# cmhungsteve/TA3N

Measured on AMD Instinct MI355X. Metric: src+tgt videos/sec per train step, UCF->HMDB_full 5-seg TA3N, higher is better.
Workload: dtype bf16

## Files before the change

### ta3n_amd/csrc/ta3n_gemm_kernel.h

```cpp
#pragma once
#include <hip/hip_runtime.h>
#include <cstdlib>
#include <cstring>

#include <type_traits>

#include "ta3n_kernels.h"

using namespace ta3n;

namespace {

typedef float f32x16 __attribute__((ext_vector_type(16)));
typedef __attribute__((address_space(3))) void lds_void_t;

constexpr int BKC = 64;

__device__ __forceinline__ float4 zero4() { return make_float4(0.f, 0.f, 0.f, 0.f); }

__device__ __forceinline__ void glds16(const float *gsrc, unsigned lds_byte_addr) {
    unsigned keep;
    lds_byte_addr = __builtin_amdgcn_readfirstlane(lds_byte_addr);
    asm volatile("s_mov_b32 %0, m0\n\ts_mov_b32 m0, %2\n\ts_nop 0\n\tglobal_load_lds_dwordx4 %1, off\n\ts_mov_b32 m0, %0"
                 : "=&s"(keep) : "v"(gsrc), "s"(lds_byte_addr) : "memory");
// ... 464 lines not shown
                    acc = __builtin_amdgcn_mfma_f32_32x32x8bf16_1k(__builtin_bit_cast(s16x4, AH), __builtin_bit_cast(s16x4, BH), acc, 0, 0, 0);
                }
            }
        }
        return;
    }
    if (BF) {
        if (NQ % 2 == 0) {
#pragma unroll
            for (int q = 0; q < NQ; q += 2) {
                if (FULL || 4 * (wk * GPW + 2 * q) < krem) {
                    const u32x4 a = {pack_bf16(av[q][0], av[q][1]), pack_bf16(av[q][2], av[q][3]),
                                     pack_bf16(av[q + 1][0], av[q + 1][1]), pack_bf16(av[q + 1][2], av[q + 1][3])};
                    const u32x4 b = {pack_bf16(bv[q][0], bv[q][1]), pack_bf16(bv[q][2], bv[q][3]),
                                     pack_bf16(bv[q + 1][0], bv[q + 1][1]), pack_bf16(bv[q + 1][2], bv[q + 1][3])};
                    acc = __builtin_amdgcn_mfma_f32_32x32x16_bf16(__builtin_bit_cast(bf16x8, a), __builtin_bit_cast(bf16x8, b),
                                                                  acc, 0, 0, 0);
                }
            }
        } else {
#pragma unroll
            for (int q = 0; q < NQ; ++q) {
                if (FULL || 4 * (wk * GPW + 2 * q) < krem) {
                    const u32x2 a = {pack_bf16(av[q][0], av[q][1]), pack_bf16(av[q][2], av[q][3])};
                    const u32x2 b = {pack_bf16(bv[q][0], bv[q][1]), pack_bf16(bv[q][2], bv[q][3])};
                    acc = __builtin_amdgcn_mfma_f32_32x32x8bf16_1k(__builtin_bit_cast(s16x4, a), __builtin_bit_cast(s16x4, b), acc,
                                                                   0, 0, 0);
                }
            }
        }
        return;
    }
#pragma unroll
    for (int q = 0; q < NQ; ++q) {
        if (FULL || 4 * (wk * GPW + 2 * q) < krem) {
#pragma unroll
            for (int j = 0; j < 4; ++j) acc = __builtin_amdgcn_mfma_f32_32x32x2f32(av[q][j], bv[q][j], acc, 0, 0, 0);
        }
    }
}

__device__ __forceinline__ void st_pub(float *p, f32x4 v) { asm volatile("global_store_dwordx4 %0, %1, off sc0 sc1" ::"v"(p), "v"(v) : "memory"); }
__device__ __forceinline__ void st_pub(void *p, u32x2 v) { asm volatile("global_store_dwordx2 %0, %1, off sc0 sc1" ::"v"(p), "v"(v) : "memory"); }
__device__ __forceinline__ void st_pub(float *p, float v) { asm volatile("global_store_dword %0, %1, off sc0 sc1" ::"v"(p), "v"(v) : "memory"); }
__device__ __forceinline__ void st_pub(unsigned short *p, unsigned v) { asm volatile("global_store_short %0, %1, off sc0 sc1" ::"v"(p), "v"(v) : "memory"); }

__device__ __forceinline__ void store_twin4(unsigned short *tp, unsigned w0, unsigned w1, int nrem, bool vec, bool pub) {
    if (nrem >= 4 && vec) {
        if (pub) st_pub(tp, u32x2{w0, w1});
        else *reinterpret_cast<u32x2 *>(tp) = u32x2{w0, w1};
    } else {
        const unsigned short h[4] = {(unsigned short)(w0 & 0xFFFF), (unsigned short)(w0 >> 16), (unsigned short)(w1 & 0xFFFF), (unsigned short)(w1 >> 16)};
#pragma unroll
        for (int e = 0; e < 4; ++e)
            if (e < nrem) { if (pub) st_pub(tp + e, (unsigned)h[e]); else tp[e] = h[e]; }
    }
}

constexpr int CHAIN_SPIN_LIMIT = 1 << 20;
__device__ __forceinline__ void chain_wait(const Task &t, const Wait *__restrict__ waits, int *__restrict__ cnt, int tid, int knobs) {
    const int nwait = (knobs & 1024) ? 0 : t.wait_count;
    if (nwait > 0) {
        if (tid < 64) {
            for (int w0 = 0; w0 < nwait; w0 += 64) {
                const bool mine = w0 + tid < nwait;
                Wait w{0, 0};
                if (mine) w = waits[t.wait_begin + w0 + tid];
                bool ok = !mine;
                int spins = 0;
                for (;;) {
                    if (!ok) ok = ((knobs & 2048) ? __hip_atomic_fetch_add(cnt + 2 + w.counter, 0, __ATOMIC_RELAXED, __HIP_MEMORY_SCOPE_AGENT)
                                                  : __hip_atomic_load(cnt + 2 + w.counter, __ATOMIC_RELAXED, __HIP_MEMORY_SCOPE_AGENT)) >= w.target;
                    if (__all(ok)) break;
                    if (++spins > CHAIN_SPIN_LIMIT) {
                        if (tid == 0) __hip_atomic_store(cnt + 1, 1 + (int)blockIdx.x, __ATOMIC_RELAXED, __HIP_MEMORY_SCOPE_AGENT);
                        break;
                    }
                    if ((spins & 1023) == 0 && __hip_atomic_load(cnt + 1, __ATOMIC_RELAXED, __HIP_MEMORY_SCOPE_AGENT) != 0) break;
                    for (int z = 0; z < (knobs & 255); ++z) __builtin_amdgcn_s_sleep(8);
                }
            }
            if (!(knobs & 256)) __builtin_amdgcn_fence(__ATOMIC_ACQUIRE, "agent");
        }
        __syncthreads();
    }
}
__device__ __forceinline__ void chain_exit(int sig, int *__restrict__ cnt, int n_counters, int tid, int knobs) {
    if ((knobs & 512) && sig < 0) return;
    asm volatile("s_waitcnt vmcnt(0)" ::: "memory");
    __syncthreads();
    if (tid == 0) {
        if (knobs & 512) { __hip_atomic_fetch_add(cnt + 2 + sig, 1, __ATOMIC_RELAXED, __HIP_MEMORY_SCOPE_AGENT); return; }
        if (sig >= 0) {
            const int before = __hip_atomic_fetch_add(cnt + 2 + sig, 1, __ATOMIC_RELAXED, __HIP_MEMORY_SCOPE_AGENT);
            asm volatile("s_waitcnt vmcnt(0)" ::"v"(before) : "memory");
        }
        const int done = __hip_atomic_fetch_add(cnt, 1, __ATOMIC_RELAXED, __HIP_MEMORY_SCOPE_AGENT);
        if (done == (int)gridDim.x - 1) {
            for (int i = 0; i < n_counters; ++i) __hip_atomic_store(cnt + 2 + i, 0, __ATOMIC_RELAXED, __HIP_MEMORY_SCOPE_AGENT);
            __hip_atomic_store(cnt, 0, __ATOMIC_RELAXED, __HIP_MEMORY_SCOPE_AGENT);
        }
    }
}

__device__ __forceinline__ const float *base_ptr(const Ptrs &p, int base) {
    switch (base) {
        case BASE_X: return p.x;
        case BASE_P: return p.p;
        case BASE_G: return p.g;
        case BASE_P16: return p.p16;
        default: return p.ws;
    }
}

}

#ifdef TA3N_GEMM_STAMPS
#define TA3N_STAMP_SLOTS 16
#define TA3N_STAMP_FLOATS (8192 * TA3N_STAMP_SLOTS * 2)
#define GSTAMP_PTR (reinterpret_cast<unsigned long long *>(const_cast<float *>(ptrs.ws) + zeros_off - TA3N_STAMP_FLOATS))
#define GSTAMP(i) do { if (threadIdx.x == 0 && blockIdx.x < 8192) GSTAMP_PTR[blockIdx.x * TA3N_STAMP_SLOTS + (i)] = __builtin_amdgcn_s_memtime(); } while (0)
#define GSTAMP_VAL(i, v) do { if (threadIdx.x == 0 && blockIdx.x < 8192) GSTAMP_PTR[blockIdx.x * TA3N_STAMP_SLOTS + (i)] = (unsigned long long)(v); } while (0)
#define GSTAMP_W1(i, v) do { if (threadIdx.x == 64 && blockIdx.x < 8192) GSTAMP_PTR[blockIdx.x * TA3N_STAMP_SLOTS + (i)] = (unsigned long long)(v); } while (0)
#define FSTAMP_DECL unsigned long long ks_f0 = __builtin_amdgcn_s_memtime(), ks_f[4] = {0, 0, 0, 0}, ks_e = 0
#define FSTAMP(i, dep) do { asm volatile("" ::"s"(dep)); ks_f[i] = (__builtin_amdgcn_s_memtime() - ks_f0) & 0xFFFFull; } while (0)
#define ESTAMP(a, b, c) do { asm volatile("" ::"s"(a), "s"(b), "s"(c)); ks_e = __builtin_amdgcn_s_memtime(); } while (0)
#define KSTAMP_DECL unsigned long long ks_wait = 0, ks_comp = 0, ks_t = 0, ks_bnd = 0, ks_int = 0, ks_mfull = 0, ks_mlast = 0, ks_m0 = 0; int ks_n = 0
#define KSTAMP_ISSUED(acc) do { acc += (__builtin_amdgcn_s_memtime() - ks_t) + (1ull << 40); } while (0)
#define KSTAMP_COMP_BEGIN do { ks_m0 = __builtin_amdgcn_s_memtime(); } while (0)
#define KSTAMP_COMP_DONE(acc) do { acc += (__builtin_amdgcn_s_memtime() - ks_m0) + (1ull << 40); } while (0)
#define KSTAMP_BEGIN_WAIT do { ks_t = __builtin_amdgcn_s_memtime(); } while (0)
#define KSTAMP_END_WAIT do { const unsigned long long n_ = __builtin_amdgcn_s_memtime(); ks_wait += n_ - ks_t; ks_t = n_; ++ks_n; } while (0)
#define KSTAMP_END_COMP do { if (ks_t != 0) { const unsigned long long n_ = __builtin_amdgcn_s_memtime(); ks_comp += n_ - ks_t; } } while (0)
#else
#define GSTAMP(i) do { } while (0)
#define GSTAMP_VAL(i, v) do { } while (0)
#define FSTAMP_DECL ((void)0)
#define FSTAMP(i, dep) ((void)0)
#define ESTAMP(a, b, c) ((void)0)
#define KSTAMP_DECL do { } while (0)
#define KSTAMP_BEGIN_WAIT do { } while (0)
#define KSTAMP_END_WAIT do { } while (0)
#define KSTAMP_END_COMP do { } while (0)
#define KSTAMP_ISSUED(acc) do { } while (0)
#define KSTAMP_COMP_BEGIN do { } while (0)
#define KSTAMP_COMP_DONE(acc) do { } while (0)
#endif

#ifndef TA3N_SEG_FAST
#define TA3N_SEG_FAST 1
#endif
#ifndef TA3N_TASK_FAST
#define TA3N_TASK_FAST 1
#endif

#define TASK_F(f) (TASK_LANES ? static_cast<decltype(t.f)>(__builtin_amdgcn_readlane(tv, (int)(offsetof(Task, f) / 4))) : t.f)
#define TASK_A(a, i) (TASK_LANES ? __builtin_amdgcn_readlane(tv, (int)(offsetof(Task, a) / 4) + (i)) : t.a[i])
#define HYPER_F(f) (TASK_LANES ? __builtin_bit_cast(float, __builtin_amdgcn_readlane(hv, (int)(offsetof(Hyper, f) / 4))) : hh.f)
#define HYPER_U(f) (TASK_LANES ? (uint32_t)__builtin_amdgcn_readlane(hv, (int)(offsetof(Hyper, f) / 4)) : hh.f)

namespace ta3n {

template <int WM, int WN, int WK, int BF, int NS, int RM, int RN, int KV = 63>
__device__ __forceinline__ void gemm_tile(const Task &t, const Seg *__restrict__ segs, const Ptrs &ptrs, int hyper_off, int zeros_off,
                                          int twin_off, const SgdSide &side, int pair_delta, int knobs) {
    constexpr int NW = WM * WN * WK, NT = 64 * NW;
    constexpr int BM = 32 * WM * RM, BN = 32 * WN * RN;
    constexpr bool HS = BF == 5;
    constexpr int ROWF = HS ? BKC / 2 : BKC;
    constexpr int STAGE = (BM + BN) * ROWF;
    constexpr int CH = BF == 2 ? 2 * BKC : BKC;
    constexpr bool TW = BF == 2 || BF == 4 || BF == 5;
    constexpr bool PAIR = BF == 4;
    constexpr int EPI = NW * RM * RN * 32 * 36;
    constexpr int LDS_FLOATS = NS * STAGE > EPI + 4 ? NS * STAGE : EPI + 4;
    __shared__ __attribute__((aligned(16))) float lds[LDS_FLOATS];

    const int tid = threadIdx.x, lane = tid & 63;
    const int wave = __builtin_amdgcn_readfirstlane(tid >> 6);
    const unsigned lds_base = __builtin_amdgcn_readfirstlane((unsigned)(uintptr_t)(lds_void_t *)lds);
    const int li = lane & 31, lh = lane >> 5;
    const int wk = wave % WK, wn = (wave / WK) % WN, wm = wave / (WK * WN);

    GSTAMP(0);
    FSTAMP_DECL;
    constexpr bool TASK_LANES = TA3N_EXPERIMENTS == 0 && KV != 63 && (TA3N_TASK_FAST) != 0;
    static_assert(sizeof(Task) == 200 && sizeof(Task) / 4 <= 64, "a Task is 50 dwords: one per lane of a wave");
    static_assert(offsetof(Hyper, train) / 4 == 19, "the per-step scalars the tiles use are the first 20 dwords of Hyper");
    int tv = 0, hv = 0;
    if constexpr (TASK_LANES) {
        __builtin_memcpy(&tv, reinterpret_cast<const char *>(&t) + 4 * (lane < (int)(sizeof(Task) / 4) ? lane : 0), 4);
        __builtin_memcpy(&hv, reinterpret_cast<const char *>(ptrs.ws + hyper_off) + 4 * (lane < 20 ? lane : 0), 4);
        asm volatile("" ::"v"(tv), "v"(hv));
    }
    FSTAMP(0, TASK_F(epi));
    auto task_seg0 = [&]() -> Seg {
        Seg s;
        s.a_base = TASK_F(seg0.a_base); s.b_base = TASK_F(seg0.b_base); s.a_off = TASK_F(seg0.a_off); s.b_off = TASK_F(seg0.b_off);
        s.a_ld = TASK_F(seg0.a_ld); s.b_ld = TASK_F(seg0.b_ld); s.a_kmajor = TASK_F(seg0.a_kmajor); s.b_kmajor = TASK_F(seg0.b_kmajor);
        s.klen = TASK_F(seg0.klen); s.scale_kind = TASK_F(seg0.scale_kind); s.pad[0] = TASK_A(seg0.pad, 0); s.pad[1] = TASK_A(seg0.pad, 1);
        return s;
    };
    constexpr bool OPT = TA3N_EXPERIMENTS != 0 && (KV & 32) != 0;
    const bool pub = OPT && TASK_F(sig) >= 0 && !(side.p16_off == -12345);
    if (TASK_F(epi) & EPI_SGD) {
        if (side.params == nullptr) return;
        float part = 0.f;
        if (tid < 256)
            part = strided_partial_sum(ptrs.ws + side.norm_off, side.norm_n, tid, 256);
        part = wave_allreduce_sum(part);
        if (lane == 0 && wave < 4) lds[wave] = part;
        __syncthreads();
        const float total = sqrtf(((lds[0] + lds[1]) + lds[2]) + lds[3]);
        const float coef = clip_coef(total, side.clip);
        float4 *__restrict__ p4 = reinterpret_cast<float4 *>(side.params);
        float4 *__restrict__ m4 = reinterpret_cast<float4 *>(side.momentum);
        const float4 *__restrict__ g4 = reinterpret_cast<const float4 *>(ptrs.g);
        for (int i = TASK_A(pad, 0) + tid; i < TASK_A(pad, 1); i += NT) {
            const float4 p = p4[i], m = m4[i], gr = g4[i];
            float gg[4] = {gr.x, gr.y, gr.z, gr.w}, pp[4] = {p.x, p.y, p.z, p.w}, mm[4] = {m.x, m.y, m.z, m.w};
#pragma unroll
            for (int e = 0; e < 4; ++e) nesterov_sgd(pp[e], mm[e], gg[e] * coef, side.lr, side.mu, side.wd);
            if (pub) st_pub(reinterpret_cast<float *>(p4 + i), f32x4{pp[0], pp[1], pp[2], pp[3]});
            else p4[i] = make_float4(pp[0], pp[1], pp[2], pp[3]);
            m4[i] = make_float4(mm[0], mm[1], mm[2], mm[3]);
            if (side.p16_off >= 0) {
                uint2 *tw = reinterpret_cast<uint2 *>(ptrs.ws + side.p16_off) + i;
                const unsigned h0 = pack_bf16(pp[0], pp[1]), h1 = pack_bf16(pp[2], pp[3]);
                if (pub) st_pub(tw, u32x2{h0, h1});
                else *tw = make_uint2(h0, h1);
                if ((BF == 3 || BF == 4) && pair_delta) {
                    const u32x2 l = {pack_bf16_lo(pp[0], pp[1], h0), pack_bf16_lo(pp[2], pp[3], h1)};
                    if (pub) st_pub(tw + pair_delta / 2, l);
                    else tw[pair_delta / 2] = make_uint2(l[0], l[1]);
                }
            }
        }
        return;
    }
    if (TASK_F(epi) & EPI_COLSUM) {
        float *__restrict__ dst = const_cast<float *>(base_ptr(ptrs, TASK_F(c_base))) + (size_t)TASK_F(c_off);
        const float *__restrict__ src = ptrs.ws + TASK_A(pad, 0);
        float sq = 0.f;
        for (int n = TASK_F(n0) + tid; n < TASK_F(n_valid); n += NT) {
            float v = 0.f;
            const float *__restrict__ col = src + n;
            const int R = TASK_A(pad, 1);
            const size_t ld = (size_t)TASK_A(pad, 2);
            int r = 0;
#pragma unroll 1
            for (; r + 8 <= R; r += 8) {
                float x[8];
#pragma unroll
                for (int i = 0; i < 8; ++i) x[i] = col[(size_t)(r + i) * ld];
#pragma unroll
                for (int i = 0; i < 8; ++i) v += x[i];
            }
            for (; r < R; ++r) v += col[(size_t)r * ld];
            dst[n] = v;
            sq = fmaf(v, v, sq);
            if (OPT && side.p_new != nullptr && TASK_F(c_base) == BASE_G) {
                const size_t pi = (size_t)TASK_F(c_off) + n;
                float p1 = ptrs.p[pi], mm = side.momentum[pi];
                nesterov_sgd(p1, mm, v, side.lr, side.mu, side.wd);
                side.p_new[pi] = p1; side.momentum[pi] = mm;
                if (side.p16_new != nullptr) reinterpret_cast<unsigned short *>(side.p16_new)[pi] = (unsigned short)(pack_bf16(p1, 0.f) & 0xFFFF);
            }
        }
        if (TASK_F(epi) & EPI_SUMSQ) {
            sq = wave_allreduce_sum(sq);
            if (lane == 0) lds[wave] = sq;
            __syncthreads();
            if (tid == 0) {
                float tot = 0.f;
                for (int i = 0; i < NW; ++i) tot += lds[i];
                ptrs.ws[TASK_A(pad, 3)] = tot;
            }
        }
        return;
    }
    if (TASK_F(seg_count) == 0) return;
    if (TASK_F(epi) & EPI_SUMROWS8) {
        const float *__restrict__ src = ptrs.ws + TASK_A(pad, 1);
        float sacc = 0.f;
        for (int r = tid >> 3; r < TASK_A(pad, 2); r += NT / 8) sacc += src[r * 8 + (tid & 7)];
        lds[tid] = sacc;
        __syncthreads();
        if (tid < 8) {
            float v = 0.f;
            for (int i = 0; i < NT / 8; ++i) v += lds[i * 8 + tid];
            ptrs.ws[TASK_A(pad, 0) + tid] = v;
        }
        __syncthreads();
    }
    const Hyper *__restrict__ hy = reinterpret_cast<const Hyper *>(ptrs.ws + hyper_off);
    const float *__restrict__ zeros = ptrs.ws + zeros_off;
    const uint32_t epi = TASK_F(epi);
    struct HyperHead { float beta[3], gamma, lr, momentum, weight_decay, clip, p_drop_i, p_drop_v; uint32_t seed_i, seed_v; };
    const HyperHead hh = TASK_LANES ? HyperHead{} : *reinterpret_cast<const HyperHead *>(hy);
    const int h_train_mem = TASK_LANES ? 0 : hy->train;
#define HYPER_TRAIN (TASK_LANES ? __builtin_amdgcn_readlane(hv, (int)(offsetof(Hyper, train) / 4)) : h_train_mem)
    FSTAMP(1, TASK_LANES ? 0 : h_train_mem);
    auto scale_of = [&](int kind) -> float {
        switch (kind) {
            case SK_NEG_BETA_REL: return -HYPER_F(beta[0]);
            case SK_NEG_BETA_VID: return -HYPER_F(beta[1]);
// ... 255 lines not shown
                    compute_stage<BM, BN, WK, AKM, BKM, true, RS, BF, RM, RN>(acc, rs, sa, sa + BM * ROWF, ra, rb, wk, lh, CH);
                    KSTAMP_COMP_DONE(ks_mfull);
                    buf ^= 1;
                }
                stage_ready();
                const int krem = klen - (n_chunks - 1) * CH, c_scale = scale;
                ++cseg;
                const bool more = cseg < seg_end;
                if (more) {
                    open_seg(cseg);
                    issue(buf ^ 1, 0);
                    KSTAMP_ISSUED(ks_bnd);
                }
                const float *sa = lds + buf * STAGE;
                KSTAMP_COMP_BEGIN;
                compute_stage<BM, BN, WK, AKM, BKM, false, RS, BF, RM, RN>(acc, rs, sa, sa + BM * ROWF, ra, rb, wk, lh, krem);
                if (krem == CH) KSTAMP_COMP_DONE(ks_mlast);
                if (c_scale != SK_ONE) {
                    const float sc = scale_of(c_scale);
    #pragma unroll
                    for (int i = 0; i < RM; ++i)
    #pragma unroll
                        for (int j = 0; j < RN; ++j)
    #pragma unroll
                            for (int r = 0; r < 16; ++r) acc[i][j][r] *= sc;
                }
                if (cseg >= seg_end) break;
                buf ^= 1;
            }
            } else {
            OperandStream<BM, NW, TW, PAIR, HS> oa;
            OperandStream<BN, NW, TW, PAIR, HS> ob;
            constexpr int LPW = OperandStream<BM, NW, TW, PAIR, HS>::NP + OperandStream<BN, NW, TW, PAIR, HS>::NP;
            int i_seg = cseg, i_chunk = 0, i_nchunks = 0, i_klen = 0, i_buf = 0, ahead = 0;
            Seg nx = TASK_LANES ? task_seg0() : t.seg0;
            auto open_issue_seg = [&]() {
                const Seg sg = nx;
                if (i_seg + 1 < seg_end) nx = segs[i_seg + 1];
                i_klen = sg.klen; i_nchunks = (sg.klen + CH - 1) / CH; i_chunk = 0;
                oa.setup(base_ptr(ptrs, sg.a_base) + (size_t)sg.a_off, sg.a_ld, AKM, sg.klen, m0, sg.pad[0] > 0 ? sg.pad[0] : m_valid,
                         wave, lane, pair_delta);
                ob.setup(base_ptr(ptrs, sg.b_base) + (size_t)sg.b_off, sg.b_ld, BKM, sg.klen, n0, n_valid, wave, lane, pair_delta);
            };
            auto issue_one = [&]() {
                const unsigned st = lds_base + (unsigned)(i_buf * STAGE * 4);
                const int k0 = i_chunk * CH;
                oa.issue(k0, i_klen - k0, st, wave, lane, zeros);
                ob.issue(k0, i_klen - k0, st + BM * ROWF * 4, wave, lane, zeros);
                i_buf = (i_buf + 1 == NS) ? 0 : i_buf + 1;
                ++ahead;
                if (++i_chunk == i_nchunks) {
                    if (++i_seg < seg_end) open_issue_seg();
                }
            };
            auto wait_landed = [&](int younger) {
                static_assert((NS - 2) * LPW <= 63, "vmcnt is a 6-bit counter");
                KSTAMP_END_COMP;
                KSTAMP_BEGIN_WAIT;
                if (NS == 2 || younger == 0) asm volatile("s_waitcnt vmcnt(0)" ::: "memory");
                else if (NS == 3 || younger == 1) asm volatile("s_waitcnt vmcnt(%0)" ::"n"(LPW) : "memory");
                else if (NS == 4 || younger == 2) asm volatile("s_waitcnt vmcnt(%0)" ::"n"(2 * LPW) : "memory");
                else if (NS == 5 || younger == 3) asm volatile("s_waitcnt vmcnt(%0)" ::"n"(3 * LPW) : "memory");
                else asm volatile("s_waitcnt vmcnt(%0)" ::"n"(4 * LPW) : "memory");
                __builtin_amdgcn_s_barrier();
                asm volatile("" ::: "memory");
                KSTAMP_END_WAIT;
            };
            open_issue_seg();
    #pragma unroll 1
            for (int sidx = 0; sidx < NS - 1 && i_seg < seg_end; ++sidx) issue_one();
            FSTAMP(3, 0);

            int c_buf = 0;
            int c_klen_nx = TASK_F(seg0.klen), c_scale_nx = TASK_F(seg0.scale_kind);
            for (;;) {
                const int klen = c_klen_nx, c_scale = c_scale_nx;
                if (cseg + 1 < seg_end) { c_klen_nx = segs[cseg + 1].klen; c_scale_nx = segs[cseg + 1].scale_kind; }
                const int n_chunks = (klen + CH - 1) / CH;
                int c = 0;
                if (i_seg == cseg) {
                    for (; c + (NS - 1) < n_chunks; ++c) {
                        wait_landed(NS - 2);
                        const unsigned st = lds_base + (unsigned)(i_buf * STAGE * 4);
                        const int k0 = (c + NS - 1) * CH;
                        const float *sa = lds + c_buf * STAGE;
                        oa.issue(k0, klen - k0, st, wave, lane, zeros);
                        ob.issue(k0, klen - k0, st + BM * ROWF * 4, wave, lane, zeros);
                        KSTAMP_ISSUED(ks_int);
                        KSTAMP_COMP_BEGIN;
                        compute_stage<BM, BN, WK, AKM, BKM, true, RS, BF, RM, RN>(acc, rs, sa, sa + BM * ROWF, ra, rb, wk, lh, CH);
                        KSTAMP_COMP_DONE(ks_mfull);
                        i_buf = (i_buf + 1 == NS) ? 0 : i_buf + 1;
                        c_buf = (c_buf + 1 == NS) ? 0 : c_buf + 1;
                    }
                    if (++i_seg < seg_end) open_issue_seg();
                }
    #pragma unroll 1
                for (; c < n_chunks; ++c) {
                    wait_landed(ahead - 1);
#ifdef TA3N_GEMM_STAMPS
                    const bool ks_first = i_chunk == 0;
                    const int ks_ahead = ahead;
#endif
                    if (i_seg < seg_end) issue_one();
#ifdef TA3N_GEMM_STAMPS
                    if (ahead == ks_ahead) { }
                    else if (ks_first) KSTAMP_ISSUED(ks_bnd);
                    else KSTAMP_ISSUED(ks_int);
#endif
                    const float *sa = lds + c_buf * STAGE;
                    KSTAMP_COMP_BEGIN;
                    if (c < n_chunks - 1)
                        compute_stage<BM, BN, WK, AKM, BKM, true, RS, BF, RM, RN>(acc, rs, sa, sa + BM * ROWF, ra, rb, wk, lh, CH);
                    else
                        compute_stage<BM, BN, WK, AKM, BKM, false, RS, BF, RM, RN>(acc, rs, sa, sa + BM * ROWF, ra, rb, wk, lh, klen - c * CH);
#ifdef TA3N_GEMM_STAMPS
                    if (c < n_chunks - 1) KSTAMP_COMP_DONE(ks_mfull);
                    else if (klen - c * CH == CH) KSTAMP_COMP_DONE(ks_mlast);
#endif
                    c_buf = (c_buf + 1 == NS) ? 0 : c_buf + 1;
                    --ahead;
                }
                if (c_scale != SK_ONE) {
                    const float sc = scale_of(c_scale);
    #pragma unroll
                    for (int i = 0; i < RM; ++i)
    #pragma unroll
                        for (int j = 0; j < RN; ++j)
    #pragma unroll
                            for (int r = 0; r < 16; ++r) acc[i][j][r] *= sc;
                }
                if (++cseg >= seg_end) break;
            }
            }
    };
    using T_ = std::true_type;
    using F_ = std::false_type;
    {
        switch (TASK_F(seg0.a_kmajor) * 2 + TASK_F(seg0.b_kmajor)) {
            case 0: if constexpr (KVE & 1) k_loop(F_{}, F_{}, F_{}); break;
            case 1: if constexpr (KVE & 2) k_loop(F_{}, T_{}, F_{}); break;
            case 2: if constexpr (KVE & 4) k_loop(T_{}, F_{}, F_{}); break;
            default:
                if (TASK_F(epi) & EPI_ROWSUM_A) { if constexpr (KVE & 16) k_loop(T_{}, T_{}, T_{}); }
                else { if constexpr (KVE & 8) k_loop(T_{}, T_{}, F_{}); }
                break;
        }
    }

    KSTAMP_END_COMP;
    GSTAMP(2);
#ifdef TA3N_GEMM_STAMPS
    GSTAMP_VAL(8, ks_wait); GSTAMP_VAL(9, ks_comp); GSTAMP_VAL(10, ks_n);
    GSTAMP_VAL(12, ks_bnd); GSTAMP_VAL(13, ks_int); GSTAMP_VAL(14, ks_mfull); GSTAMP_VAL(15, ks_mlast);
#endif
    __syncthreads();
    GSTAMP(3);
#pragma unroll
    for (int i = 0; i < RM; ++i)
#pragma unroll
        for (int j = 0; j < RN; ++j) {
            float *cs = lds + ((wave * RM + i) * RN + j) * (32 * 36);
#pragma unroll
            for (int r = 0; r < 16; ++r) {
                const int row = (r & 3) + 8 * (r >> 2) + 4 * lh;
                cs[row * 36 + li] = acc[i][j][r];
            }
        }
    __syncthreads();
    GSTAMP(4);

    const float *__restrict__ split_other = nullptr;
    if (OPT && (epi & EPI_SPLITK)) {
        int &split_ticket = *reinterpret_cast<int *>(&lds[EPI]);
        const int half = TASK_A(pad, 2) - 1;
        float *mine = ptrs.ws + TASK_A(pad, 0) + (size_t)half * (BM * BN);
        constexpr int ITER_S = (BM * BN / 4 + NT - 1) / NT;
#pragma unroll
        for (int it = 0; it < ITER_S; ++it) {
            const int idx = tid + it * NT;
            if (idx < BM * BN / 4) {
                const int r = idx / (BN / 4), c4 = (idx % (BN / 4)) * 4;
                const int br = r >> 5, bc = c4 >> 5;
                const int slot0 = ((((br / RM) * WN + (bc / RN)) * WK) * RM + (br % RM)) * RN + (bc % RN);
                float4 v4 = zero4();
#pragma unroll
                for (int q = 0; q < WK; ++q) {
                    const float4 part = *reinterpret_cast<const float4 *>(&lds[(slot0 + q * RM * RN) * (32 * 36) + (r & 31) * 36 + (c4 & 31)]);
                    v4.x += part.x; v4.y += part.y; v4.z += part.z; v4.w += part.w;
                }
                st_pub(mine + (size_t)r * BN + c4, f32x4{v4.x, v4.y, v4.z, v4.w});
            }
        }
        asm volatile("s_waitcnt vmcnt(0)" ::: "memory");
        __syncthreads();
        int *ticket = reinterpret_cast<int *>(ptrs.ws + TASK_A(pad, 1));
        if (tid == 0) split_ticket = __hip_atomic_fetch_add(ticket, 1, __ATOMIC_RELAXED, __HIP_MEMORY_SCOPE_AGENT);
        __syncthreads();
        if (split_ticket == 0) return;
        if (tid == 0) __hip_atomic_store(ticket, 0, __ATOMIC_RELAXED, __HIP_MEMORY_SCOPE_AGENT);
        split_other = ptrs.ws + TASK_A(pad, 0) + (size_t)(1 - half) * (BM * BN);
    }
    const float alpha = scale_of(TASK_F(alpha_kind));
    const float gamma = scale_of(TASK_F(gamma_kind));
    const bool drop_on = (epi & (EPI_DROP_I | EPI_DROP_V)) && HYPER_TRAIN != 0;
    const uint32_t dseed = (epi & EPI_DROP_I) ? HYPER_U(seed_i) : HYPER_U(seed_v);
    const float dp = (epi & EPI_DROP_I) ? HYPER_F(p_drop_i) : HYPER_F(p_drop_v);
    const uint32_t doff = drop_on ? (uint32_t)TASK_F(pad2) : 0u;
    float *__restrict__ cbase = const_cast<float *>(base_ptr(ptrs, TASK_F(c_base))) + (size_t)TASK_F(c_off);
    const EpiOperands eo = PF_IT > 0 ? eo_early : epi_operands();
    const int nfan = eo.nfan;
    const bool c_vec = ((TASK_F(c_off) | TASK_F(c_ld)) & 3) == 0;
    const bool upd = OPT && side.p_new != nullptr && TASK_F(c_base) == BASE_G;
    float sumsq = 0.f;
    ESTAMP(alpha, gamma, TASK_F(c_ld));
    constexpr int ITER = (BM * BN / 4 + NT - 1) / NT;
    constexpr int UNR = ITER <= 4 ? ITER : 2;
#pragma unroll UNR
    for (int it = 0; it < ITER; ++it) {
        const int idx = tid + it * NT;
        if (idx >= BM * BN / 4) break;
        const int r = idx / (BN / 4);
        const int c4 = (idx % (BN / 4)) * 4;
        const int br = r >> 5, bc = c4 >> 5;
        const int slot0 = ((((br / RM) * WN + (bc / RN)) * WK) * RM + (br % RM)) * RN + (bc % RN);
        const int m = m0 + r, n = n0 + c4;
        const bool row_ok = m < m_valid;
        const int nrem = row_ok ? n_valid - n : 0;
        float av[4] = {0.f, 0.f, 0.f, 0.f}, mv[4] = {1.f, 1.f, 1.f, 1.f};
        float fm[3][4] = {{0.f, 0.f, 0.f, 0.f}, {0.f, 0.f, 0.f, 0.f}, {0.f, 0.f, 0.f, 0.f}};
        if constexpr (PF_IT > 0) {
#pragma unroll
            for (int e = 0; e < 4; ++e) { av[e] = add_e[PF_IT > 0 ? it : 0][e]; mv[e] = aux_e[PF_IT > 0 ? it : 0][e]; asm volatile("" : "+v"(mv[e])); }
        } else {
            fetch_add_aux(eo, av, mv, m, n, nrem);
        }
        if constexpr (PF_FAN) {
#pragma unroll
            for (int f = 0; f < 3; ++f)
#pragma unroll
                for (int e = 0; e < 4; ++e) { fm[f][e] = fan_e[f][e]; asm volatile("" : "+v"(fm[f][e])); }
        } else if constexpr (EPI_EARLY) {
            fetch_fan(eo, fm, m, n, nrem);
        }
        float up[4] = {0.f, 0.f, 0.f, 0.f}, um[4] = {0.f, 0.f, 0.f, 0.f};
        if (upd_early) {
#pragma unroll
            for (int e = 0; e < 4; ++e) { up[e] = up_e[UPD_PREFETCH ? it : 0][e]; um[e] = um_e[UPD_PREFETCH ? it : 0][e]; }
        } else if (upd && nrem > 0) {
            const size_t pi = (size_t)TASK_F(c_off) + (size_t)m * TASK_F(c_ld) + n;
            if (nrem >= 4 && c_vec) {
                const float4 q4 = *reinterpret_cast<const float4 *>(ptrs.p + pi), r4 = *reinterpret_cast<const float4 *>(side.momentum + pi);
                up[0] = q4.x; up[1] = q4.y; up[2] = q4.z; up[3] = q4.w; um[0] = r4.x; um[1] = r4.y; um[2] = r4.z; um[3] = r4.w;
            } else {
#pragma unroll
                for (int e = 0; e < 4; ++e) if (e < nrem) { up[e] = ptrs.p[pi + e]; um[e] = side.momentum[pi + e]; }
            }
        }
        float other4[4] = {0.f, 0.f, 0.f, 0.f};
        if (split_other != nullptr) {
            const float *op = split_other + (size_t)r * BN + c4;
#pragma unroll
            for (int e = 0; e < 4; ++e) other4[e] = __hip_atomic_load(op + e, __ATOMIC_RELAXED, __HIP_MEMORY_SCOPE_AGENT);
        }
        float4 v4 = zero4();
#pragma unroll
        for (int q = 0; q < WK; ++q) {
            const float4 part = *reinterpret_cast<const float4 *>(&lds[(slot0 + q * RM * RN) * (32 * 36) + (r & 31) * 36 + (c4 & 31)]);
            v4.x += part.x; v4.y += part.y; v4.z += part.z; v4.w += part.w;
        }
        if (split_other != nullptr) { v4.x += other4[0]; v4.y += other4[1]; v4.z += other4[2]; v4.w += other4[3]; }
#ifdef TA3N_GEMM_STAMPS
        if (it == 0) {
            asm volatile("s_waitcnt lgkmcnt(0)" ::: "memory");
            const unsigned long long now_ = __builtin_amdgcn_s_memtime();
            GSTAMP_W1(11, (now_ & 0xFFFFFFFFFFFFull) | (((now_ - ks_e) & 0xFFFFull) << 48));
        }
#endif
        float v[4] = {v4.x, v4.y, v4.z, v4.w};
#pragma unroll
        for (int e = 0; e < 4; ++e) {
            float x = (v[e] + ebias[e]) * alpha + av[e];
            if (epi & EPI_RELU) x = fmaxf(x, 0.f);
            x = mv[e] > 0.f ? x : 0.f;
            if (drop_on) x *= keep_mask(dseed, (uint32_t)(m * TASK_F(drop_ld) + n + e) + doff, dp);
            v[e] = x * gamma;
        }
        if (nrem <= 0) continue;
#pragma unroll
        for (int e = 0; e < 4; ++e)
            if (e < nrem) sumsq = fmaf(v[e], v[e], sumsq);
        float *cp = cbase + (size_t)m * TASK_F(c_ld) + n;
        if (epi & EPI_TWIN_ONLY) {
        } else if (nrem >= 4 && c_vec) {
            if (pub) st_pub(cp, f32x4{v[0], v[1], v[2], v[3]});
            else *reinterpret_cast<float4 *>(cp) = make_float4(v[0], v[1], v[2], v[3]);
        } else {
#pragma unroll
            for (int e = 0; e < 4; ++e)
                if (e < nrem) { if (pub) st_pub(cp + e, v[e]); else cp[e] = v[e]; }
        }
        if (upd) {
            const size_t pi = (size_t)TASK_F(c_off) + (size_t)m * TASK_F(c_ld) + n;
            float pn[4];
#pragma unroll
            for (int e = 0; e < 4; ++e) {
                pn[e] = up[e];
                nesterov_sgd(pn[e], um[e], v[e], side.lr, side.mu, side.wd);
            }
            if (nrem >= 4 && c_vec) {
                *reinterpret_cast<float4 *>(side.p_new + pi) = make_float4(pn[0], pn[1], pn[2], pn[3]);
                *reinterpret_cast<float4 *>(side.momentum + pi) = make_float4(um[0], um[1], um[2], um[3]);
                if (side.p16_new != nullptr)
                    *reinterpret_cast<u32x2 *>(reinterpret_cast<unsigned short *>(side.p16_new) + pi) = u32x2{pack_bf16(pn[0], pn[1]), pack_bf16(pn[2], pn[3])};
            } else {
#pragma unroll
                for (int e = 0; e < 4; ++e)
                    if (e < nrem) {
                        side.p_new[pi + e] = pn[e]; side.momentum[pi + e] = um[e];
                        if (side.p16_new != nullptr) reinterpret_cast<unsigned short *>(side.p16_new)[pi + e] = (unsigned short)(pack_bf16(pn[e], 0.f) & 0xFFFF);
                    }
            }
        }
        if (epi & EPI_TWIN16) {
            unsigned short *tp = reinterpret_cast<unsigned short *>(ptrs.ws + twin_off) + ((size_t)TASK_F(c_off) + (size_t)m * TASK_F(c_ld) + n);
            const unsigned lo = pack_bf16(v[0], v[1]), hi = pack_bf16(v[2], v[3]);
            store_twin4(tp, lo, hi, nrem, c_vec, pub);
            if ((BF == 3 || BF == 4) && pair_delta)
                store_twin4(tp + 2 * (size_t)pair_delta, pack_bf16_lo(v[0], v[1], lo), pack_bf16_lo(v[2], v[3], hi), nrem, c_vec, pub);
        }
        if (nfan > 0) {
            const bool fan_vec = nrem >= 4 && (TASK_F(fan_ld) & 3) == 0;
            if constexpr (!EPI_EARLY) fetch_fan(eo, fm, m, n, nrem);
#pragma unroll
            for (int f = 0; f < 3; ++f) {
                if (f < nfan) {
                    float *op = ptrs.ws + (size_t)TASK_A(fan_out_off, f) + (size_t)m * TASK_F(fan_ld) + n;
                    float ov[4];
#pragma unroll
                    for (int e = 0; e < 4; ++e) ov[e] = (e < nrem && fm[f][e] > 0.f) ? v[e] : 0.f;
                    if (epi & EPI_TWIN_ONLY_FAN) {
                    } else if (fan_vec && (TASK_A(fan_out_off, f) & 3) == 0) {
                        if (pub) st_pub(op, f32x4{ov[0], ov[1], ov[2], ov[3]});
                        else *reinterpret_cast<float4 *>(op) = make_float4(ov[0], ov[1], ov[2], ov[3]);
                    } else {
#pragma unroll
                        for (int e = 0; e < 4; ++e)
                            if (e < nrem) { if (pub) st_pub(op + e, ov[e]); else op[e] = ov[e]; }
                    }
                    if (epi & EPI_TWIN16_FAN) {
                        unsigned short *tp = reinterpret_cast<unsigned short *>(ptrs.ws + twin_off) +
                                             ((size_t)TASK_A(fan_out_off, f) + (size_t)m * TASK_F(fan_ld) + n);
                        const unsigned lo = pack_bf16(ov[0], ov[1]), hi = pack_bf16(ov[2], ov[3]);
                        const bool fvec = ((TASK_A(fan_out_off, f) | TASK_F(fan_ld)) & 3) == 0;
                        store_twin4(tp, lo, hi, nrem, fvec, pub);
                        if ((BF == 3 || BF == 4) && pair_delta)
                            store_twin4(tp + 2 * (size_t)pair_delta, pack_bf16_lo(ov[0], ov[1], lo), pack_bf16_lo(ov[2], ov[3], hi), nrem, fvec, pub);
                    }
                }
            }
        }
    }
    if (epi & EPI_ROWSUM_A) {
        __syncthreads();
        if (wn == 0) {
#pragma unroll
            for (int i = 0; i < RM; ++i) lds[(wk * 2 + lh) * BM + ra + 32 * i] = rs[i];
        }
        __syncthreads();
        if (tid < BM) {
            float b = 0.f;
#pragma unroll
            for (int i = 0; i < 2 * WK; ++i) b += lds[i * BM + tid];
            if (m0 + tid < m_valid) {
                const_cast<float *>(base_ptr(ptrs, TASK_F(bias_base)))[(size_t)TASK_F(bias_off) + m0 + tid] = b;
                sumsq = fmaf(b, b, sumsq);
                if (upd && TASK_F(bias_base) == BASE_G) {
                    const size_t pi = (size_t)TASK_F(bias_off) + m0 + tid;
                    float p1 = ptrs.p[pi], mm = side.momentum[pi];
                    nesterov_sgd(p1, mm, b, side.lr, side.mu, side.wd);
                    side.p_new[pi] = p1; side.momentum[pi] = mm;
                    if (side.p16_new != nullptr) reinterpret_cast<unsigned short *>(side.p16_new)[pi] = (unsigned short)(pack_bf16(p1, 0.f) & 0xFFFF);
                }
            }
        }
    }
    GSTAMP(5);
#if defined(TA3N_GEMM_STAMPS) && TA3N_GEMM_STAMPS == 1
    GSTAMP_VAL(6, (unsigned long long)TASK_F(cost) | ks_f[0] << 24 | ks_f[1] << 40);
    GSTAMP_VAL(7, (unsigned long long)TASK_F(seg_count) | ks_f[2] << 16 | ks_f[3] << 32);
#endif
    if (epi & EPI_SUMSQ) {
        __syncthreads();
        sumsq = wave_allreduce_sum(sumsq);
        if (lane == 0) lds[wave] = sumsq;
        __syncthreads();
        if (tid == 0) {
            float tot = 0.f;
            for (int i = 0; i < NW; ++i) tot += lds[i];
            ptrs.ws[TASK_A(pad, 3)] = tot;
        }
    }
}

#undef TASK_F
#undef TASK_A
#undef HYPER_F
#undef HYPER_U
#undef HYPER_TRAIN

template <int WM, int WN, int WK, int BF, int NS, int RM, int RN, int KV = 63>
__global__ __launch_bounds__(64 * WM * WN * WK) void gemm_tiles(const Task *__restrict__ tasks, const Seg *__restrict__ segs,
                                                                 Ptrs ptrs, int hyper_off, int zeros_off, int twin_off, SgdSide side,
                                                                 const Wait *__restrict__ waits, int chain_off, int chain_n, int knobs,
                                                                 int pair_delta) {
    int *cnt = reinterpret_cast<int *>(ptrs.ws + (chain_off >= 0 ? chain_off : 0));
    if (TA3N_EXPERIMENTS != 0 && chain_off >= 0) {
        const Task &t = tasks[blockIdx.x];
#if defined(TA3N_GEMM_STAMPS) && TA3N_GEMM_STAMPS == 2
        GSTAMP(6);
#endif
        chain_wait(t, waits, cnt, (int)threadIdx.x, knobs);
        gemm_tile<WM, WN, WK, BF, NS, RM, RN, KV>(t, segs, ptrs, hyper_off, zeros_off, twin_off, side, pair_delta, knobs);
        chain_exit(t.sig, cnt, chain_n, (int)threadIdx.x, knobs);
#if defined(TA3N_GEMM_STAMPS) && TA3N_GEMM_STAMPS == 2
        GSTAMP(7);
#endif
        return;
    }
    gemm_tile<WM, WN, WK, BF, NS, RM, RN, KV>(tasks[blockIdx.x], segs, ptrs, hyper_off, zeros_off, twin_off, side, pair_delta, knobs);
}

#define TA3N_TILE_CONFIGS(X) X(1, 1, 4) X(1, 1, 8) X(2, 1, 2) X(1, 2, 2) X(2, 1, 4) X(1, 2, 4) X(2, 2, 1) X(2, 2, 2)

#define TA3N_BLOCKED_CONFIGS(X) X(2, 2, 2, 2, 2, 2) X(2, 2, 1, 2, 2, 2) X(2, 2, 2, 1, 2, 2) X(2, 2, 2, 1, 2, 3) X(2, 2, 2, 2, 1, 2) X(2, 2, 2, 2, 1, 3)

#define TA3N_INSTANTIATE(wm, wn, wk)                                                                        \
    template __global__ void gemm_tiles<wm, wn, wk, 0, 2, 1, 1>(const Task *, const Seg *, Ptrs, int, int, int, SgdSide, const Wait *, int, int, int, int); \
    template __global__ void gemm_tiles<wm, wn, wk, 1, 2, 1, 1>(const Task *, const Seg *, Ptrs, int, int, int, SgdSide, const Wait *, int, int, int, int); \
    template __global__ void gemm_tiles<wm, wn, wk, 1, 3, 1, 1>(const Task *, const Seg *, Ptrs, int, int, int, SgdSide, const Wait *, int, int, int, int); \
    template __global__ void gemm_tiles<wm, wn, wk, 2, 2, 1, 1>(const Task *, const Seg *, Ptrs, int, int, int, SgdSide, const Wait *, int, int, int, int); \
    template __global__ void gemm_tiles<wm, wn, wk, 2, 3, 1, 1>(const Task *, const Seg *, Ptrs, int, int, int, SgdSide, const Wait *, int, int, int, int); \
    template __global__ void gemm_tiles<wm, wn, wk, 3, 2, 1, 1>(const Task *, const Seg *, Ptrs, int, int, int, SgdSide, const Wait *, int, int, int, int); \
    template __global__ void gemm_tiles<wm, wn, wk, 3, 3, 1, 1>(const Task *, const Seg *, Ptrs, int, int, int, SgdSide, const Wait *, int, int, int, int); \
    template __global__ void gemm_tiles<wm, wn, wk, 4, 2, 1, 1>(const Task *, const Seg *, Ptrs, int, int, int, SgdSide, const Wait *, int, int, int, int); \
    template __global__ void gemm_tiles<wm, wn, wk, 4, 3, 1, 1>(const Task *, const Seg *, Ptrs, int, int, int, SgdSide, const Wait *, int, int, int, int);
#if TA3N_EXPERIMENTS
#define TA3N_HS_CONFIGS(X) X(2, 2, 2, 2, 2, 3) X(2, 2, 2, 2, 2, 4) X(2, 2, 2, 1, 1, 3) X(2, 2, 2, 1, 1, 4) X(2, 2, 1, 3, 2, 3) X(2, 2, 1, 4, 2, 3) X(2, 2, 1, 2, 2, 2)
#else
#define TA3N_HS_CONFIGS(X) X(2, 2, 2, 2, 2, 3) X(2, 2, 2, 1, 1, 3) X(2, 2, 1, 2, 2, 2)
#endif
#define TA3N_INSTANTIATE_HS(wm, wn, wk, rm, rn, ns) \
    template __global__ void gemm_tiles<wm, wn, wk, 5, ns, rm, rn>(const Task *, const Seg *, Ptrs, int, int, int, SgdSide, const Wait *, int, int, int, int);

#define TA3N_INSTANTIATE_BLOCKED(wm, wn, wk, rm, rn, ns) \
    template __global__ void gemm_tiles<wm, wn, wk, 2, ns, rm, rn>(const Task *, const Seg *, Ptrs, int, int, int, SgdSide, const Wait *, int, int, int, int);


#define TA3N_KIND_CONFIGS(X) X(1, 2, 4, 2, 3, 1) X(1, 2, 4, 1, 2, 26) X(2, 2, 2, 2, 2, 26) \
                             X(2, 1, 4, 4, 3, 1) X(1, 2, 4, 3, 2, 26) X(1, 2, 2, 4, 2, 26)
#define TA3N_INSTANTIATE_KIND(wm, wn, wk, bf, ns, kv) \
    template __global__ void gemm_tiles<wm, wn, wk, bf, ns, 1, 1, kv>(const Task *, const Seg *, Ptrs, int, int, int, SgdSide, const Wait *, int, int, int, int);


}
```

Measured before the change: 2.080 million.

## Hoist GEMM epilogue setup and LDS partial loads, drop tail barriers in specialised kernels

For kind-specialised GEMM kernels, the epilogue scalars, per-pass index and address arithmetic, and fan-mask fetches are computed before the barrier that follows the accumulator spill, so they overlap with LDS writes. The LDS partial-sum reads and aux fetches are issued together at the top of each pass. The row-sum and sum-of-squares reductions use LDS regions past the epilogue staging area, which lets them drop a __syncthreads each. The cost is higher register pressure from the precomputed per-pass state, plus static asserts that limit the path to tiles stored in one or two full passes.

```diff
diff --git a/ta3n_amd/csrc/ta3n_gemm_kernel.h b/ta3n_amd/csrc/ta3n_gemm_kernel.h
--- a/ta3n_amd/csrc/ta3n_gemm_kernel.h
+++ b/ta3n_amd/csrc/ta3n_gemm_kernel.h
@@ -640,6 +640,9 @@
 #endif
 #ifndef TA3N_TASK_FAST
 #define TA3N_TASK_FAST 1
+#endif
+#ifndef TA3N_TAIL_FAST
+#define TA3N_TAIL_FAST 1
 #endif
 
 #define TASK_F(f) (TASK_LANES ? static_cast<decltype(t.f)>(__builtin_amdgcn_readlane(tv, (int)(offsetof(Task, f) / 4))) : t.f)
@@ -1201,8 +1204,38 @@
     GSTAMP(2);
 #ifdef TA3N_GEMM_STAMPS
     GSTAMP_VAL(8, ks_wait); GSTAMP_VAL(9, ks_comp); GSTAMP_VAL(10, ks_n);
+#if TA3N_GEMM_STAMPS != 3
     GSTAMP_VAL(12, ks_bnd); GSTAMP_VAL(13, ks_int); GSTAMP_VAL(14, ks_mfull); GSTAMP_VAL(15, ks_mlast);
 #endif
+#endif
+    constexpr bool TAIL_FAST = TA3N_EXPERIMENTS == 0 && KV != 63 && (TA3N_TAIL_FAST) != 0;
+    constexpr int ITER = (BM * BN / 4 + NT - 1) / NT;
+    constexpr int UNR = ITER <= 4 ? ITER : 2;
+    static_assert(!TAIL_FAST || (ITER <= 2 && ITER * NT == BM * BN / 4), "the kind-specialised kernels store their tile in one or two full passes");
+    constexpr int SQ_AT = EPI + 4, RS_AT = EPI + 4 + 8;
+    static_assert(!TAIL_FAST || (NW <= 8 && RS_AT + 2 * WK * BM <= LDS_FLOATS), "the reduction words fit behind the epilogue staging");
+    float alpha_e = 1.f, gamma_e = 1.f, dp_e = 0.f;
+    bool drop_on_e = false, c_vec_e = false;
+    uint32_t dseed_e = 0u, doff_e = 0u;
+    float *cbase_e = nullptr;
+    struct PassSetup { int m, n, nrem, lds_at4; uint32_t drop_at; size_t c_at, fan_at; };
+    auto pass_setup = [&](int it) -> PassSetup {
+        const int idx = tid + it * NT;
+        const int r = idx / (BN / 4);
+        const int c4 = (idx % (BN / 4)) * 4;
+        const int br = r >> 5, bc = c4 >> 5;
+        const int slot0 = ((((br / RM) * WN + (bc / RN)) * WK) * RM + (br % RM)) * RN + (bc % RN);
+        const int m = m0 + r, n = n0 + c4;
+        const bool row_ok = m < m_valid;
+        const int nrem = row_ok ? n_valid - n : 0;
+        return PassSetup{m, n, nrem, slot0 * (32 * 9) + (r & 31) * 9 + ((c4 & 31) >> 2), (uint32_t)(m * TASK_F(drop_ld) + n),
+                         (size_t)m * TASK_F(c_ld) + n, (size_t)m * TASK_F(fan_ld) + n};
+    };
+    PassSetup ps_early[TAIL_FAST ? ITER : 1] = {};
+    constexpr bool FAN_TAIL = TAIL_FAST && EPI_EARLY && !PF_FAN;
+    static_assert(!FAN_TAIL || PF_IT == ITER, "eo_early is set");
+    float fan_t[FAN_TAIL ? ITER : 1][3][4];
+
     __syncthreads();
     GSTAMP(3);
 #pragma unroll
@@ -1216,6 +1249,37 @@
                 cs[row * 36 + li] = acc[i][j][r];
             }
         }
+    if constexpr (TAIL_FAST) {
+        alpha_e = scale_of(TASK_F(alpha_kind));
+        gamma_e = scale_of(TASK_F(gamma_kind));
+        drop_on_e = (epi & (EPI_DROP_I | EPI_DROP_V)) && HYPER_TRAIN != 0;
+        dseed_e = (epi & EPI_DROP_I) ? HYPER_U(seed_i) : HYPER_U(seed_v);
+        dp_e = (epi & EPI_DROP_I) ? HYPER_F(p_drop_i) : HYPER_F(p_drop_v);
+        doff_e = drop_on_e ? (uint32_t)TASK_F(pad2) : 0u;
+        cbase_e = const_cast<float *>(base_ptr(ptrs, TASK_F(c_base))) + (size_t)TASK_F(c_off);
+        c_vec_e = ((TASK_F(c_off) | TASK_F(c_ld)) & 3) == 0;
+        asm volatile("" : "+v"(alpha_e), "+v"(gamma_e), "+s"(dseed_e), "+s"(dp_e), "+s"(doff_e), "+s"(cbase_e));
+#pragma unroll
+        for (int it = 0; it < ITER; ++it) {
+            ps_early[it] = pass_setup(it);
+            asm volatile("" : "+v"(ps_early[it].m), "+v"(ps_early[it].n), "+v"(ps_early[it].nrem), "+v"(ps_early[it].lds_at4), "+v"(ps_early[it].drop_at),
+                         "+v"(ps_early[it].c_at), "+v"(ps_early[it].fan_at));
+        }
+        if constexpr (FAN_TAIL) {
+#pragma unroll
+            for (int it = 0; it < ITER; ++it) {
+#pragma unroll
+                for (int f = 0; f < 3; ++f)
+#pragma unroll
+                    for (int e = 0; e < 4; ++e) fan_t[it][f][e] = 0.f;
+                fetch_fan(eo_early, fan_t[it], ps_early[it].m, ps_early[it].n, ps_early[it].nrem);
+            }
+        }
+    }
+#if defined(TA3N_GEMM_STAMPS) && TA3N_GEMM_STAMPS == 3
+    asm volatile("s_waitcnt lgkmcnt(0)" ::: "memory");
+    GSTAMP(12);
+#endif
     __syncthreads();
     GSTAMP(4);
 
@@ -1250,21 +1314,19 @@
         if (tid == 0) __hip_atomic_store(ticket, 0, __ATOMIC_RELAXED, __HIP_MEMORY_SCOPE_AGENT);
         split_other = ptrs.ws + TASK_A(pad, 0) + (size_t)(1 - half) * (BM * BN);
     }
-    const float alpha = scale_of(TASK_F(alpha_kind));
-    const float gamma = scale_of(TASK_F(gamma_kind));
-    const bool drop_on = (epi & (EPI_DROP_I | EPI_DROP_V)) && HYPER_TRAIN != 0;
-    const uint32_t dseed = (epi & EPI_DROP_I) ? HYPER_U(seed_i) : HYPER_U(seed_v);
-    const float dp = (epi & EPI_DROP_I) ? HYPER_F(p_drop_i) : HYPER_F(p_drop_v);
-    const uint32_t doff = drop_on ? (uint32_t)TASK_F(pad2) : 0u;
-    float *__restrict__ cbase = const_cast<float *>(base_ptr(ptrs, TASK_F(c_base))) + (size_t)TASK_F(c_off);
+    const float alpha = TAIL_FAST ? alpha_e : scale_of(TASK_F(alpha_kind));
+    const float gamma = TAIL_FAST ? gamma_e : scale_of(TASK_F(gamma_kind));
+    const bool drop_on = TAIL_FAST ? drop_on_e : (epi & (EPI_DROP_I | EPI_DROP_V)) && HYPER_TRAIN != 0;
+    const uint32_t dseed = TAIL_FAST ? dseed_e : (epi & EPI_DROP_I) ? HYPER_U(seed_i) : HYPER_U(seed_v);
+    const float dp = TAIL_FAST ? dp_e : (epi & EPI_DROP_I) ? HYPER_F(p_drop_i) : HYPER_F(p_drop_v);
+    const uint32_t doff = TAIL_FAST ? doff_e : drop_on ? (uint32_t)TASK_F(pad2) : 0u;
+    float *__restrict__ cbase = TAIL_FAST ? cbase_e : const_cast<float *>(base_ptr(ptrs, TASK_F(c_base))) + (size_t)TASK_F(c_off);
     const EpiOperands eo = PF_IT > 0 ? eo_early : epi_operands();
     const int nfan = eo.nfan;
-    const bool c_vec = ((TASK_F(c_off) | TASK_F(c_ld)) & 3) == 0;
+    const bool c_vec = TAIL_FAST ? c_vec_e : ((TASK_F(c_off) | TASK_F(c_ld)) & 3) == 0;
     const bool upd = OPT && side.p_new != nullptr && TASK_F(c_base) == BASE_G;
     float sumsq = 0.f;
     ESTAMP(alpha, gamma, TASK_F(c_ld));
-    constexpr int ITER = (BM * BN / 4 + NT - 1) / NT;
-    constexpr int UNR = ITER <= 4 ? ITER : 2;
 #pragma unroll UNR
     for (int it = 0; it < ITER; ++it) {
         const int idx = tid + it * NT;
@@ -1273,23 +1335,34 @@
         const int c4 = (idx % (BN / 4)) * 4;
         const int br = r >> 5, bc = c4 >> 5;
         const int slot0 = ((((br / RM) * WN + (bc / RN)) * WK) * RM + (br % RM)) * RN + (bc % RN);
-        const int m = m0 + r, n = n0 + c4;
+        const PassSetup ps = ps_early[TAIL_FAST ? it : 0];
+        const int m = TAIL_FAST ? ps.m : m0 + r, n = TAIL_FAST ? ps.n : n0 + c4;
         const bool row_ok = m < m_valid;
-        const int nrem = row_ok ? n_valid - n : 0;
+        const int nrem = TAIL_FAST ? ps.nrem : row_ok ? n_valid - n : 0;
         float av[4] = {0.f, 0.f, 0.f, 0.f}, mv[4] = {1.f, 1.f, 1.f, 1.f};
         float fm[3][4] = {{0.f, 0.f, 0.f, 0.f}, {0.f, 0.f, 0.f, 0.f}, {0.f, 0.f, 0.f, 0.f}};
+#if defined(TA3N_GEMM_STAMPS) && TA3N_GEMM_STAMPS == 3
+        if (it == 0) GSTAMP(13);
+#endif
+        float4 part_e[TAIL_FAST ? WK : 1];
+        if constexpr (TAIL_FAST) {
+            if constexpr (PF_IT == 0) fetch_add_aux(eo, av, mv, m, n, nrem);
+#pragma unroll
+            for (int q = 0; q < WK; ++q) part_e[TAIL_FAST ? q : 0] = reinterpret_cast<const float4 *>(lds)[ps.lds_at4 + q * RM * RN * (32 * 9)];
+            __builtin_amdgcn_sched_barrier(0);
+        }
         if constexpr (PF_IT > 0) {
 #pragma unroll
             for (int e = 0; e < 4; ++e) { av[e] = add_e[PF_IT > 0 ? it : 0][e]; mv[e] = aux_e[PF_IT > 0 ? it : 0][e]; asm volatile("" : "+v"(mv[e])); }
-        } else {
+        } else if constexpr (!TAIL_FAST) {
             fetch_add_aux(eo, av, mv, m, n, nrem);
         }
-        if constexpr (PF_FAN) {
+        if constexpr (PF_FAN || FAN_TAIL) {
 #pragma unroll
             for (int f = 0; f < 3; ++f)
 #pragma unroll
-                for (int e = 0; e < 4; ++e) { fm[f][e] = fan_e[f][e]; asm volatile("" : "+v"(fm[f][e])); }
-        } else if constexpr (EPI_EARLY) {
+                for (int e = 0; e < 4; ++e) { fm[f][e] = PF_FAN ? fan_e[f][e] : fan_t[FAN_TAIL ? it : 0][f][e]; asm volatile("" : "+v"(fm[f][e])); }
+        } else if constexpr (EPI_EARLY && !TAIL_FAST) {
             fetch_fan(eo, fm, m, n, nrem);
         }
         float up[4] = {0.f, 0.f, 0.f, 0.f}, um[4] = {0.f, 0.f, 0.f, 0.f};
@@ -1315,7 +1388,7 @@
         float4 v4 = zero4();
 #pragma unroll
         for (int q = 0; q < WK; ++q) {
-            const float4 part = *reinterpret_cast<const float4 *>(&lds[(slot0 + q * RM * RN) * (32 * 36) + (r & 31) * 36 + (c4 & 31)]);
+            const float4 part = TAIL_FAST ? part_e[TAIL_FAST ? q : 0] : *reinterpret_cast<const float4 *>(&lds[(slot0 + q * RM * RN) * (32 * 36) + (r & 31) * 36 + (c4 & 31)]);
             v4.x += part.x; v4.y += part.y; v4.z += part.z; v4.w += part.w;
         }
         if (split_other != nullptr) { v4.x += other4[0]; v4.y += other4[1]; v4.z += other4[2]; v4.w += other4[3]; }
@@ -1332,14 +1405,17 @@
             float x = (v[e] + ebias[e]) * alpha + av[e];
             if (epi & EPI_RELU) x = fmaxf(x, 0.f);
             x = mv[e] > 0.f ? x : 0.f;
-            if (drop_on) x *= keep_mask(dseed, (uint32_t)(m * TASK_F(drop_ld) + n + e) + doff, dp);
+            if (drop_on) x *= keep_mask(dseed, TAIL_FAST ? ps.drop_at + (uint32_t)e + doff : (uint32_t)(m * TASK_F(drop_ld) + n + e) + doff, dp);
             v[e] = x * gamma;
         }
+#if defined(TA3N_GEMM_STAMPS) && TA3N_GEMM_STAMPS == 3
+        if (it == 0) GSTAMP(14);
+#endif
         if (nrem <= 0) continue;
 #pragma unroll
         for (int e = 0; e < 4; ++e)
             if (e < nrem) sumsq = fmaf(v[e], v[e], sumsq);
-        float *cp = cbase + (size_t)m * TASK_F(c_ld) + n;
+        float *cp = TAIL_FAST ? cbase + ps.c_at : cbase + (size_t)m * TASK_F(c_ld) + n;
         if (epi & EPI_TWIN_ONLY) {
         } else if (nrem >= 4 && c_vec) {
             if (pub) st_pub(cp, f32x4{v[0], v[1], v[2], v[3]});
@@ -1372,7 +1448,7 @@
             }
         }
         if (epi & EPI_TWIN16) {
-            unsigned short *tp = reinterpret_cast<unsigned short *>(ptrs.ws + twin_off) + ((size_t)TASK_F(c_off) + (size_t)m * TASK_F(c_ld) + n);
+            unsigned short *tp = reinterpret_cast<unsigned short *>(ptrs.ws + twin_off) + (TAIL_FAST ? (size_t)TASK_F(c_off) + ps.c_at : (size_t)TASK_F(c_off) + (size_t)m * TASK_F(c_ld) + n);
             const unsigned lo = pack_bf16(v[0], v[1]), hi = pack_bf16(v[2], v[3]);
             store_twin4(tp, lo, hi, nrem, c_vec, pub);
             if ((BF == 3 || BF == 4) && pair_delta)
@@ -1384,7 +1460,7 @@
 #pragma unroll
             for (int f = 0; f < 3; ++f) {
                 if (f < nfan) {
-                    float *op = ptrs.ws + (size_t)TASK_A(fan_out_off, f) + (size_t)m * TASK_F(fan_ld) + n;
+                    float *op = TAIL_FAST ? ptrs.ws + (size_t)TASK_A(fan_out_off, f) + ps.fan_at : ptrs.ws + (size_t)TASK_A(fan_out_off, f) + (size_t)m * TASK_F(fan_ld) + n;
                     float ov[4];
 #pragma unroll
                     for (int e = 0; e < 4; ++e) ov[e] = (e < nrem && fm[f][e] > 0.f) ? v[e] : 0.f;
@@ -1399,7 +1475,7 @@
                     }
                     if (epi & EPI_TWIN16_FAN) {
                         unsigned short *tp = reinterpret_cast<unsigned short *>(ptrs.ws + twin_off) +
-                                             ((size_t)TASK_A(fan_out_off, f) + (size_t)m * TASK_F(fan_ld) + n);
+                                             (TAIL_FAST ? (size_t)TASK_A(fan_out_off, f) + ps.fan_at : (size_t)TASK_A(fan_out_off, f) + (size_t)m * TASK_F(fan_ld) + n);
                         const unsigned lo = pack_bf16(ov[0], ov[1]), hi = pack_bf16(ov[2], ov[3]);
                         const bool fvec = ((TASK_A(fan_out_off, f) | TASK_F(fan_ld)) & 3) == 0;
                         store_twin4(tp, lo, hi, nrem, fvec, pub);
@@ -1411,16 +1487,17 @@
         }
     }
     if (epi & EPI_ROWSUM_A) {
-        __syncthreads();
+        float *rsw = lds + (TAIL_FAST ? RS_AT : 0);
+        if constexpr (!TAIL_FAST) __syncthreads();
         if (wn == 0) {
 #pragma unroll
-            for (int i = 0; i < RM; ++i) lds[(wk * 2 + lh) * BM + ra + 32 * i] = rs[i];
+            for (int i = 0; i < RM; ++i) rsw[(wk * 2 + lh) * BM + ra + 32 * i] = rs[i];
         }
         __syncthreads();
         if (tid < BM) {
             float b = 0.f;
 #pragma unroll
-            for (int i = 0; i < 2 * WK; ++i) b += lds[i * BM + tid];
+            for (int i = 0; i < 2 * WK; ++i) b += rsw[i * BM + tid];
             if (m0 + tid < m_valid) {
                 const_cast<float *>(base_ptr(ptrs, TASK_F(bias_base)))[(size_t)TASK_F(bias_off) + m0 + tid] = b;
                 sumsq = fmaf(b, b, sumsq);
@@ -1435,21 +1512,25 @@
         }
     }
     GSTAMP(5);
-#if defined(TA3N_GEMM_STAMPS) && TA3N_GEMM_STAMPS == 1
+#if defined(TA3N_GEMM_STAMPS) && (TA3N_GEMM_STAMPS == 1 || TA3N_GEMM_STAMPS == 3)
     GSTAMP_VAL(6, (unsigned long long)TASK_F(cost) | ks_f[0] << 24 | ks_f[1] << 40);
     GSTAMP_VAL(7, (unsigned long long)TASK_F(seg_count) | ks_f[2] << 16 | ks_f[3] << 32);
 #endif
     if (epi & EPI_SUMSQ) {
-        __syncthreads();
+        float *sqw = lds + (TAIL_FAST ? SQ_AT : 0);
+        if constexpr (!TAIL_FAST) __syncthreads();
         sumsq = wave_allreduce_sum(sumsq);
-        if (lane == 0) lds[wave] = sumsq;
+        if (lane == 0) sqw[wave] = sumsq;
         __syncthreads();
         if (tid == 0) {
             float tot = 0.f;
-            for (int i = 0; i < NW; ++i) tot += lds[i];
+            for (int i = 0; i < NW; ++i) tot += sqw[i];
             ptrs.ws[TASK_A(pad, 3)] = tot;
         }
     }
+#if defined(TA3N_GEMM_STAMPS) && TA3N_GEMM_STAMPS == 3
+    GSTAMP(15);
+#endif
 }
 
 #undef TASK_F
```

Measured after the change: 2.079 million. About the same (-0.0%).
